# kezakool/flair-for-aigle

Measured on AMD Instinct MI355X. Metric: 512x512x5 tiles/sec (train fwd+bwd+AdamW), U-Net ResNet-34, 19 classes, higher is better.
Workload: dtype bf16; 1 GPU; synthetic 512x512x5 tiles, 19-class U-Net (ResNet-34 encoder), batch 32 per GPU, train step (BASELINE.json configs[1]); global_batch=32, tile=512, parallelism=dp1

## Files before the change

flair-for-aigle_amd/csrc/conv_wgrad.hip:

```cpp
#include "ffa_common.h"
#include <hip/hip_ext.h>

#include <stdlib.h>

#ifndef FFA_WGRAD_TRACE
#define FFA_WGRAD_TRACE 0
#endif
#if FFA_WGRAD_TRACE
__device__ long long ffa_wgrad_trace_buf[64 * 256];
#define FFA_WTRACE(slot_)                                                                   \
  if (trace_on) {                                                                           \
    if (trace_n < 256)                                                                      \
      ffa_wgrad_trace_buf[(blockIdx.y * gridDim.x + blockIdx.x) * 256 + trace_n] =          \
          (long long)(slot_) << 56 | (__builtin_readcyclecounter() & 0xFFFFFFFFFFFFFFLL);    \
    ++trace_n;                                                                              \
  }
#else
#define FFA_WTRACE(slot_)
#endif

struct WgradArgs {
  const void* x;
  const void* dy;
  float* slabs;
  int B, Hi, Wi, Ci;
  int Ho, Wo, Co;
  int pad;
  int tiles_x, tiles_y, npt;
  int ncob, ncib, nsplit;
  const void* x2;
  int C1;
  int CoT, CiT;
  const float* pro_sc;
  const float* pro_sh;
  int ci_real;
};

template <int KH, int KW, int STRIDE, int RG, int WCO, int WCI, int WK, int TH, int TW, int EB>
struct WgradGeom {
  static constexpr int NTHR = 64 * WCO * WCI * WK;
  static constexpr int NPX = TH * TW;
  static constexpr bool ONE = (KH == 1 && KW == 1);
  static constexpr int LS = ONE ? 1 : STRIDE;
  static constexpr int GSTEP = ONE ? STRIDE : 1;
  static constexpr int NRG = KH / RG;
  static constexpr int IH = (TH - 1) * LS + RG;
  static constexpr int IW = (TW - 1) * LS + KW;
  static constexpr int TAPS = RG * KW;
  static constexpr int ROWB = 32 * EB;
  static constexpr int PARTS = ROWB / 16;
  static constexpr int DY_BYTES = WCO * NPX * ROWB;
  static constexpr int IN_BYTES = WCI * IH * IW * ROWB;
  static constexpr int STAGE_BYTES = DY_BYTES + IN_BYTES;
  static constexpr bool MERGE = (WK > 1) && (WCO * WCI == 4 || KH == 7);
  static constexpr int MERGE_BYTES = MERGE ? WCO * WCI * (WK - 1) * TAPS * 16 * 64 * 4 : 0;
  static constexpr int LDS_BYTES = STAGE_BYTES > MERGE_BYTES ? STAGE_BYTES : MERGE_BYTES;
  static constexpr int DY_PIECES = WCO * NPX * PARTS;
  static constexpr int IN_PIECES = WCI * IH * IW * PARTS;
  static constexpr int NDP = (DY_PIECES + NTHR - 1) / NTHR;
  static constexpr int NIP = (IN_PIECES + NTHR - 1) / NTHR;
  static constexpr int KSTEPS = NPX / 16;
  static_assert(TW % 16 == 0, "a 16-pixel k-step must stay inside one tile row");
  static_assert(KSTEPS % WK == 0, "k-steps must divide over the k-split waves");
  static_assert(LDS_BYTES <= 160 * 1024, "LDS budget");
};

__device__ __forceinline__ ffa_s16x4 lds_read_tr16(const unsigned char* p) {
  return __builtin_amdgcn_ds_read_tr16_b64_v4i16(
// ... 1002 lines not shown

  float* slab = a.slabs + (size_t)blockIdx.x * a.CoT * 9 * a.CiT;
#pragma unroll
  for (int mt = 0; mt < MT; ++mt)
#pragma unroll
    for (int nt = 0; nt < NT; ++nt)
#pragma unroll
      for (int tp = 0; tp < 9; ++tp)
#pragma unroll
        for (int i = 0; i < 4; ++i) {
          const int co = mt * 16 + 4 * kg + i, ci = nt * 16 + li;
          slab[((size_t)co * 9 + tp) * a.CiT + ci] = acc[mt][nt][tp][i];
        }
}


template <int TW_>
struct Wg64Geom {
  static constexpr int TW = TW_, TH = 256 / TW_, IH = TH + 2, IW = TW + 2;
  static constexpr int RS = 32 / TW;
  static constexpr int XP = IH * IW * 8, YP = TH * TW * 8;
  static constexpr int PIECES = XP + YP;
  static constexpr int NHW = (PIECES + 511) / 512;
  static constexpr int X_BYTES = XP * 16;
  static constexpr int SLOT = PIECES * 16;
  static constexpr int ACC_BYTES = 144 * 64 * 4;
  static constexpr int LDS_BYTES = (2 * SLOT > 4 * ACC_BYTES) ? 2 * SLOT : 4 * ACC_BYTES;
  static_assert(TW == 32 || TW == 16, "tile width");
  static_assert(LDS_BYTES <= 160 * 1024, "LDS budget");
};

__device__ __forceinline__ int wg64_phi(int px) { return ((px >> 1) & 1) | (((px >> 3) & 1) << 1); }

template <int TW>
__global__ void __launch_bounds__(512) conv3x3_wgrad64_kernel(WgradArgs a) {
  using G = Wg64Geom<TW>;
  __shared__ __align__(16) unsigned char smem[G::LDS_BYTES];
  const int tid = threadIdx.x;
  const int lane = tid & 63;
  const int wave = __builtin_amdgcn_readfirstlane(tid >> 6);
  const int kgp = wave >> 2;
  const int wco = (wave >> 1) & 1, wci = wave & 1;
  const int li = lane & 15, kg = lane >> 4;
  const int cib = blockIdx.x % a.ncib, cob = blockIdx.x / a.ncib;
  const int co0 = cob * 64, ci0 = cib * 64;
  const int split = blockIdx.y;

  const bool two = a.C1 > 0;
  const bool from_lo = two && ci0 < a.C1;
  const size_t xpb = (size_t)(!two ? a.Ci : from_lo ? a.C1 : a.Ci - a.C1) * 2, ypb = (size_t)a.Co * 2;
  const int xW = from_lo ? a.Wi / 2 : a.Wi, xH = from_lo ? a.Hi / 2 : a.Hi;
  int pinfo[G::NHW];
#pragma unroll
  for (int k = 0; k < G::NHW; ++k) {
    const int p = tid + k * 512;
    if (p < G::XP) {
      const int q = p >> 3, yy = q / G::IW, xx = q % G::IW, sl = (p & 7) ^ (2 * wg64_phi(xx));
      const int py = from_lo ? ((yy - 1) >> 1) + 1 : yy, px = from_lo ? ((xx - 1) >> 1) + 1 : xx;
      pinfo[k] = ((((py * xW + px) * (int)xpb) >> 4) + sl) << 13 | (yy << 6) | xx;
    } else if (p < G::PIECES) {
      const int q = (p - G::XP) >> 3, yy = q / G::TW, xx = q % G::TW, sl = (p & 7) ^ (2 * wg64_phi(xx));
      pinfo[k] = ((((yy * a.Wo + xx) * (int)ypb) >> 4) + sl) << 13 | (1 << 12) | (yy << 6) | xx;
    } else {
      pinfo[k] = 1 << 11;
    }
  }
  const unsigned char* x_b = (two && !from_lo) ? static_cast<const unsigned char*>(a.x2) + (ci0 - a.C1) * 2
                                               : static_cast<const unsigned char*>(a.x) + ci0 * 2;
  const unsigned char* dy_b = static_cast<const unsigned char*>(a.dy) + co0 * 2;
  const unsigned char* zero = reinterpret_cast<const unsigned char*>(ffa_wgthin_zero16);
  const bool has_tail = (G::PIECES % 512 == 0) || (wave * 64 + (G::NHW - 1) * 512 < G::PIECES);

  auto tile_origin = [&](int t, int& b, int& oy0, int& ox0) {
    const int tx = t % a.tiles_x;
    const int t2 = t / a.tiles_x;
    oy0 = (t2 % a.tiles_y) * G::TH;
    b = t2 / a.tiles_y;
    ox0 = tx * G::TW;
  };
// ... 98 lines not shown
        __builtin_amdgcn_sched_barrier(0);
      }
      slot ^= 1;
    }
  }
  asm volatile("s_waitcnt vmcnt(0)\n\ts_barrier" ::: "memory");

  float* red = reinterpret_cast<float*>(smem) + (size_t)(wave & 3) * 144 * 64 + lane;
  if (kgp == 1) {
    int o = 0;
#pragma unroll
    for (int mt = 0; mt < 2; ++mt)
#pragma unroll
      for (int nt = 0; nt < 2; ++nt)
#pragma unroll
        for (int tp = 0; tp < 9; ++tp)
#pragma unroll
          for (int i = 0; i < 4; ++i) red[(o++) * 64] = acc[mt][nt][tp][i];
  }
  __syncthreads();
  if (kgp == 1) return;
  {
    int o = 0;
#pragma unroll
    for (int mt = 0; mt < 2; ++mt)
#pragma unroll
      for (int nt = 0; nt < 2; ++nt)
#pragma unroll
        for (int tp = 0; tp < 9; ++tp)
#pragma unroll
          for (int i = 0; i < 4; ++i) acc[mt][nt][tp][i] += red[(o++) * 64];
  }
  float* slab = a.slabs + (size_t)split * a.CoT * 9 * a.CiT;
#pragma unroll
  for (int mt = 0; mt < 2; ++mt)
#pragma unroll
    for (int nt = 0; nt < 2; ++nt)
#pragma unroll
      for (int tp = 0; tp < 9; ++tp)
#pragma unroll
        for (int i = 0; i < 4; ++i) {
          const int co = co0 + wco * 32 + mt * 16 + 4 * kg + i, ci = ci0 + wci * 32 + nt * 16 + li;
          slab[((size_t)co * 9 + tp) * a.CiT + ci] = acc[mt][nt][tp][i];
        }
}


struct WgStem8Geom {
  static constexpr int TH = 8, TW = 32, IH = 2 * TH + 5, IWC = 72;
  static constexpr int XP = IH * IWC, YP = TH * TW * 8;
  static constexpr int PIECES = XP + YP;
  static constexpr int NHW = (PIECES + 511) / 512;
  static constexpr int X_BYTES = XP * 16;
  static constexpr int SLOT = PIECES * 16;
  static constexpr int ACC_BYTES = 112 * 64 * 4;
  static constexpr int LDS_BYTES = (2 * SLOT > 4 * ACC_BYTES) ? 2 * SLOT : 4 * ACC_BYTES;
  static_assert(LDS_BYTES <= 160 * 1024, "LDS budget");
};

__global__ void __launch_bounds__(512) stem_wgrad8_kernel(WgradArgs a) {
  using G = WgStem8Geom;
  __shared__ __align__(16) unsigned char smem[G::LDS_BYTES];
  const int tid = threadIdx.x;
  const int lane = tid & 63;
  const int wave = __builtin_amdgcn_readfirstlane(tid >> 6);
  const int kgp = wave >> 2;
  const int sp = wave & 3;
  const int li = lane & 15, kg = lane >> 4;
  const int split = blockIdx.y;

  int pinfo[G::NHW];
#pragma unroll
  for (int k = 0; k < G::NHW; ++k) {
    const int p = tid + k * 512;
    if (p < G::XP) {
      const int hy = p / G::IWC, hx = p % G::IWC;
      pinfo[k] = (hx < 2 * G::TW + 5) ? (((hy * a.Wi + hx) * 2) << 14 | (hy << 7) | hx) : (1 << 12);
// ... 103 lines not shown
#pragma unroll
      for (int r = 0; r < 7; ++r)
#pragma unroll
        for (int i = 0; i < 4; ++i) red[(o++) * 64] = acc[mt][r][i];
  }
  __syncthreads();
  if (kgp == 1) return;
  {
    int o = 0;
#pragma unroll
    for (int mt = 0; mt < 4; ++mt)
#pragma unroll
      for (int r = 0; r < 7; ++r)
#pragma unroll
        for (int i = 0; i < 4; ++i) acc[mt][r][i] += red[(o++) * 64];
  }
  const int s = 2 * sp + (li >> 3), ch = li & 7;
  if (s < 7) {
#pragma unroll
    for (int mt = 0; mt < 4; ++mt)
#pragma unroll
      for (int r = 0; r < 7; ++r)
#pragma unroll
        for (int i = 0; i < 4; ++i) {
          const int co = mt * 16 + 4 * kg + i;
          a.slabs[(((size_t)split * a.CoT + co) * 49 + r * 7 + s) * 16 + ch] = acc[mt][r][i];
        }
  }
}


struct WgradPlan {
  int wco, wci, wk, th, tw, rg, nsplit, ncob, ncib, CoT, CiT, npt, tiles_x, tiles_y, ring, nslab, stem, thin;
};

static bool wgrad_plan(int dtype, int kh, int kw, int stride, int Co, int Ci, int B, int Ho, int Wo, WgradPlan* p,
                       bool allow_ring = true, bool allow_thin = true) {
  const bool s1 = (kh == 3 && kw == 3 && stride == 1);
  const bool s2 = (kh == 3 && kw == 3 && stride == 2);
  const bool one = (kh == 1 && kw == 1 && (stride == 1 || stride == 2));
  const bool stem = (kh == 7 && kw == 7 && stride == 2);
  if (!(s1 || s2 || one || stem)) return false;
  const bool f32 = (dtype == FFA_F32);
  p->rg = stem ? 1 : kh;
  p->wk = 1;
  p->thin = 0;
  {
    const char* tw_ = getenv("FFA_THIN_WGRAD");
    if (allow_thin && s1 && !f32 && !(tw_ && tw_[0] == '0') && (Co == 16 || Co == 32) && (Ci == 16 || Ci == 32)) {
      p->thin = 1;
      p->th = 8; p->tw = 32;
      p->wco = p->wci = 1;
      p->ncob = p->ncib = 1;
      p->CoT = Co; p->CiT = Ci;
      p->tiles_x = ffa_cdiv(Wo, 32);
      p->tiles_y = ffa_cdiv(Ho, 8);
      p->npt = B * p->tiles_x * p->tiles_y;
      p->ring = 0; p->stem = 0;
      p->nsplit = p->npt < 512 ? p->npt : 512;
      p->nslab = p->nsplit;
      return true;
    }
  }
  if (s1) {
    p->tw = (Wo >= 32) ? 32 : 16;
    p->th = (Wo >= 32) ? 4 : 8;
// ... 46 lines not shown
    p->CoT = Co;
    p->CiT = 16;
    ns = 256 / (Co / 64);
    if (ns > p->npt) ns = p->npt;
    if (ns < 1) ns = 1;
  }
  p->nsplit = ns;
  const bool merge = p->wk > 1 && (p->wco * p->wci == 4 || stem);
  p->nslab = merge ? ns : ns * p->wk;
  return true;
}

extern "C" long long ffa_conv_wgrad_workspace_bytes(int dtype, int kh, int kw, int stride, int Co, int Ci, int B, int Ho,
                                                    int Wo) {
  WgradPlan p, q;
  if (!wgrad_plan(dtype, kh, kw, stride, Co, Ci, B, Ho, Wo, &p)) return FFA_ERR_UNSUPPORTED;
  long long need = (long long)p.nslab * p.CoT * kh * kw * p.CiT * (long long)sizeof(float);
  if (p.thin) {
    wgrad_plan(dtype, kh, kw, stride, Co, Ci, B, Ho, Wo, &q, true, false);
    const long long other = (long long)q.nslab * q.CoT * kh * kw * q.CiT * (long long)sizeof(float);
    if (other > need) need = other;
  }
  return need;
}

template <typename T, int KH, int KW, int STRIDE, int RG, int WCO, int WCI, int WK, int TH, int TW, bool PRO = false>
static void launch_wgrad_cfg(const WgradArgs& a, int nrg, hipStream_t stream) {
  dim3 grid(a.ncob * a.ncib * nrg, a.nsplit);
  hipLaunchKernelGGL((conv_wgrad_kernel<T, KH, KW, STRIDE, RG, WCO, WCI, WK, TH, TW, PRO>), grid,
                     dim3(64 * WCO * WCI * WK), 0, stream, a);
}

template <typename T>
static int launch_wgrad(const WgradArgs& a, const WgradPlan& p, int kh, int kw, int stride, hipStream_t stream) {
  constexpr bool F32 = (sizeof(T) == 4);
  const bool wide = (p.tw == 32);
  if constexpr (!F32) {
    if (p.thin) {
      const bool up = a.C1 > 0, pro = a.pro_sc != nullptr;
#define FFA_WGTHIN(CI_, CO_)                                                                                     \
  if (a.Ci == CI_ && a.Co == CO_) {                                                                              \
    if (up && pro) hipLaunchKernelGGL((conv3x3_thin_wgrad_kernel<CI_, CO_, true, true>), dim3(a.nsplit), dim3(256), 0, stream, a);   \
    else if (up) hipLaunchKernelGGL((conv3x3_thin_wgrad_kernel<CI_, CO_, true, false>), dim3(a.nsplit), dim3(256), 0, stream, a);    \
    else if (pro) hipLaunchKernelGGL((conv3x3_thin_wgrad_kernel<CI_, CO_, false, true>), dim3(a.nsplit), dim3(256), 0, stream, a);   \
    else hipLaunchKernelGGL((conv3x3_thin_wgrad_kernel<CI_, CO_, false, false>), dim3(a.nsplit), dim3(256), 0, stream, a);           \
    return ffa_check_launch("conv3x3_thin_wgrad");                                                               \
  }
      FFA_WGTHIN(16, 16)
      FFA_WGTHIN(16, 32)
      FFA_WGTHIN(32, 16)
      FFA_WGTHIN(32, 32)
#undef FFA_WGTHIN
      ffa_set_error("conv_wgrad: no thin kernel for pitches %d / %d", a.Ci, a.Co);
      return FFA_ERR_UNSUPPORTED;
    }
    if (p.ring) {
      dim3 grid(a.ncob * a.ncib, a.nsplit);
      if (wide) hipLaunchKernelGGL((conv_wgrad_ring_kernel<4, 32>), grid, dim3(256), 0, stream, a);
      else hipLaunchKernelGGL((conv_wgrad_ring_kernel<8, 16>), grid, dim3(256), 0, stream, a);
      return ffa_check_launch("conv_wgrad_ring");
    }
  }
  if (kh == 3 && stride == 1) {
#define FFA_WG_S1(WCO_, WCI_, WK_, THW_, THN_)                                               \
  if (p.wco == WCO_ && p.wci == WCI_ && p.wk == WK_) {                                       \
    if (wide) launch_wgrad_cfg<T, 3, 3, 1, 3, WCO_, WCI_, WK_, THW_, 32>(a, 1, stream);      \
    else launch_wgrad_cfg<T, 3, 3, 1, 3, WCO_, WCI_, WK_, THN_, 16>(a, 1, stream);           \
    return ffa_check_launch("conv_wgrad");                                                   \
  }
    if constexpr (F32) {
      FFA_WG_S1(2, 1, 1, 4, 8)
      FFA_WG_S1(1, 1, 1, 4, 8)
    } else {
      if (a.pro_sc) {
        if (!(p.wco == 2 && p.wci == 2 && p.wk == 2) || a.C1 > 0) {
          ffa_set_error("conv_wgrad: no prologue for this channel configuration");
          return FFA_ERR_UNSUPPORTED;
        }
        if (wide) launch_wgrad_cfg<T, 3, 3, 1, 3, 2, 2, 2, 8, 32, true>(a, 1, stream);
        else launch_wgrad_cfg<T, 3, 3, 1, 3, 2, 2, 2, 16, 16, true>(a, 1, stream);
        return ffa_check_launch("conv_wgrad");
      }
      {
        const char* e64 = getenv("FFA_WGRAD64");
        const int ih = wide ? 10 : 18, iw = wide ? 34 : 18;
        if (!(e64 && e64[0] == '0') && p.wco == 2 && p.wci == 2 && p.wk == 2 && p.th == (wide ? 8 : 16) && a.C1 % 64 == 0 &&
            (a.C1 == 0 || (a.Hi % 2 == 0 && a.Wi % 2 == 0)) && a.pad == 1 && a.Co % 64 == 0 && a.Ci % 64 == 0 &&
            ((long long)ih * a.Wi + iw) * 2 * (a.Ci > a.Co ? a.Ci : a.Co) < (1LL << 23)) {
          hipEvent_t ts, te;
          const dim3 grid(a.ncob * a.ncib, a.nsplit);
          const bool timed = ffa_ktime_next(FFA_KT_WGRAD64, &ts, &te);
          if (wide) {
            if (timed) hipExtLaunchKernelGGL(conv3x3_wgrad64_kernel<32>, grid, dim3(512), 0, stream, ts, te, 0, a);
            else hipLaunchKernelGGL(conv3x3_wgrad64_kernel<32>, grid, dim3(512), 0, stream, a);
          } else {
            if (timed) hipExtLaunchKernelGGL(conv3x3_wgrad64_kernel<16>, grid, dim3(512), 0, stream, ts, te, 0, a);
            else hipLaunchKernelGGL(conv3x3_wgrad64_kernel<16>, grid, dim3(512), 0, stream, a);
          }
          return ffa_check_launch("conv3x3_wgrad64");
        }
      }
      FFA_WG_S1(2, 2, 2, 8, 16)
      FFA_WG_S1(2, 1, 2, 4, 8)
      FFA_WG_S1(1, 2, 2, 4, 8)
      if (p.wco == 1 && p.wci == 1 && p.wk == 4 && (p.th == 8 && wide || p.th == 16 && !wide)) {
        if (wide) launch_wgrad_cfg<T, 3, 3, 1, 3, 1, 1, 4, 8, 32>(a, 1, stream);
        else launch_wgrad_cfg<T, 3, 3, 1, 3, 1, 1, 4, 16, 16>(a, 1, stream);
        return ffa_check_launch("conv_wgrad");
      }
      FFA_WG_S1(1, 1, 4, 4, 8)
    }
#undef FFA_WG_S1
  } else if (kh == 3 && stride == 2) {
    launch_wgrad_cfg<T, 3, 3, 2, 3, 2, F32 ? 1 : 2, 1, 4, 16>(a, 1, stream);
    return ffa_check_launch("conv_wgrad");
  } else if (kh == 1 && stride == 2) {
    launch_wgrad_cfg<T, 1, 1, 2, 1, 2, F32 ? 1 : 2, 1, 4, 16>(a, 1, stream);
    return ffa_check_launch("conv_wgrad");
  } else if (kh == 1 && stride == 1) {
    launch_wgrad_cfg<T, 1, 1, 1, 1, 2, F32 ? 1 : 2, 1, 4, 16>(a, 1, stream);
    return ffa_check_launch("conv_wgrad");
  } else if (kh == 7) {
    if constexpr (!F32) {
// ... 24 lines not shown
              "conv_wgrad: the prologue is for bf16 3x3 stride-1 pad-1 layers");
  FFA_REQUIRE(dtype == FFA_BF16 || dtype == FFA_F32, "conv_wgrad: bad dtype");
  FFA_REQUIRE(x && dy && dw_oihw && workspace, "conv_wgrad: null pointer");
  FFA_REQUIRE(Ci % 8 == 0 && Co % 8 == 0, "conv_wgrad: channel pitch must be a multiple of 8");
  FFA_REQUIRE(Co_real <= Co && Ci_real <= Ci, "conv_wgrad: real channels exceed pitch");
  WgradPlan p;
  const bool thin_ok = pad == 1 && (C1 == 0 || (C1 == Ci && x2 == nullptr));
  if (!wgrad_plan(dtype, kh, kw, stride, Co, Ci, B, Ho, Wo, &p, pad == 1 && C1 == 0, thin_ok)) {
    ffa_set_error("conv_wgrad: unsupported kernel %dx%d stride %d", kh, kw, stride);
    return FFA_ERR_UNSUPPORTED;
  }
  if (C1 > 0 && !p.thin) {
    if (C1 % (32 * p.wci) != 0) {
      ffa_set_error("conv_wgrad_upcat: C1 = %d is not a multiple of the block's %d input channels", C1, 32 * p.wci);
      return FFA_ERR_UNSUPPORTED;
    }
  }
  const long long need = (long long)p.nslab * p.CoT * kh * kw * p.CiT * (long long)sizeof(float);
  if (workspace_bytes < need) {
    ffa_set_error("conv_wgrad: workspace too small (%lld < %lld)", workspace_bytes, need);
    return FFA_ERR_WORKSPACE;
  }
  WgradArgs a;
  a.x = x; a.dy = dy; a.slabs = static_cast<float*>(workspace);
  a.x2 = x2; a.C1 = C1;
  a.pro_sc = pro_scale; a.pro_sh = pro_shift;
  a.ci_real = Ci_real;
  a.B = B; a.Hi = Hi; a.Wi = Wi; a.Ci = Ci;
  a.Ho = Ho; a.Wo = Wo; a.Co = Co;
  a.pad = pad;
  a.tiles_x = p.tiles_x; a.tiles_y = p.tiles_y; a.npt = p.npt;
  a.ncob = p.ncob; a.ncib = p.ncib; a.nsplit = p.nsplit;
  a.CoT = p.CoT; a.CiT = p.CiT;
  int rc = (dtype == FFA_BF16) ? launch_wgrad<ffa_bf16>(a, p, kh, kw, stride, stream)
                               : launch_wgrad<float>(a, p, kh, kw, stride, stream);
  if (rc != FFA_OK) return rc;
  const long long total = (long long)Co_real * kh * kw * ((Ci_real + 3) / 4);
  const char* rv = getenv("FFA_WG_REDUCE_V1");
  const bool reduce_v1 = rv && rv[0] == '1';
  const int cq = (Ci_real + 3) / 4;
  const int v2_blocks = Co_real * ffa_cdiv(cq, p.nslab > 8 ? 8 : 64);
  if (kh == 3 && kw == 3 && !reduce_v1 && v2_blocks >= 512) {
    if (p.nslab > 8) {
      hipLaunchKernelGGL(wgrad_reduce3x3_kernel<32>, dim3(v2_blocks), dim3(256), 0, stream,
                         (const float*)workspace, dw_oihw, p.nslab, p.CoT, p.CiT, Co_real, Ci_real, accumulate);
    } else {
      hipLaunchKernelGGL(wgrad_reduce3x3_kernel<4>, dim3(v2_blocks), dim3(256), 0, stream,
                         (const float*)workspace, dw_oihw, p.nslab, p.CoT, p.CiT, Co_real, Ci_real, accumulate);
    }
    return ffa_check_launch("wgrad_reduce3x3");
  }
  if (p.nslab > 8) {
    long long g = (total + 7) / 8;
    if (g > 4096) g = 4096;
    hipLaunchKernelGGL(wgrad_reduce_kernel<32>, dim3((int)g), dim3(256), 0, stream, (const float*)workspace, dw_oihw,
                       p.nslab, p.CoT, p.CiT, Co_real, Ci_real, kh * kw, accumulate);
  } else {
    long long g = (total + 63) / 64;
    if (g > 4096) g = 4096;
    hipLaunchKernelGGL(wgrad_reduce_kernel<4>, dim3((int)g), dim3(256), 0, stream, (const float*)workspace, dw_oihw,
                       p.nslab, p.CoT, p.CiT, Co_real, Ci_real, kh * kw, accumulate);
  }
  return ffa_check_launch("wgrad_reduce");
}

extern "C" int ffa_conv_wgrad(int dtype, const void* x, const void* dy, float* dw_oihw, int B, int Hi, int Wi, int Ci,
                              int Ho, int Wo, int Co, int Co_real, int Ci_real, int kh, int kw, int stride, int pad,
                              int accumulate, void* workspace, long long workspace_bytes, hipStream_t stream) {
  return wgrad_impl(dtype, x, nullptr, 0, dy, dw_oihw, B, Hi, Wi, Ci, Ho, Wo, Co, Co_real, Ci_real, kh, kw, stride, pad,
// ... 85 lines not shown
```

flair-for-aigle_amd/flairhip/lib.py:

```python
from __future__ import annotations

import ctypes as C
import os

_HERE = os.path.dirname(os.path.abspath(__file__))
LIB_PATH = os.environ.get("FLAIRHIP_LIB") or os.path.join(_HERE, "libflairhip.so")

BF16 = 0
F32 = 1
BCO_RING = 0x1000
BCO_THIN = 0x2000
BCO_STEM = 0x8000
ERR_UNSUPPORTED = -2


class FlairHipError(RuntimeError):
    pass


class Tile(C.Structure):
    _fields_ = [
        ("left", C.c_double), ("bottom", C.c_double), ("right", C.c_double), ("top", C.c_double),
        ("x0", C.c_double), ("y0", C.c_double), ("x1", C.c_double), ("y1", C.c_double),
        ("row", C.c_longlong), ("col", C.c_longlong),
# ... 28 lines not shown
    "ffa_pack_desc_fill_cols": (_i, [_p, _p, _p, _p] + [_i] * 12),
    "ffa_pack_conv_weights_batched": (_i, [_i, _p, _i, _p]),
    "ffa_conv2d": (_i, [_i, _p, _p, _p, _p, _p] + [_i] * 15 + [_p]),
    "ffa_conv_stat_rows": (_ll, [_i, _i, _i, _i, _i]),
    "ffa_conv_plan": (_i, [_i] * 7),
    "ffa_ring_conv3x3": (_i, [_i, _p, _p, _p, _p, _p, _p, _p, _p] + [_i] * 7 + [_p]),
    "ffa_ring_stat_rows": (_ll, [_i, _i, _i, _i]),
    "ffa_ring_pack": (_i, [_i, _p, _p, _p, _i, _i, _i, _i, _i, _p]),
    "ffa_conv2d_pro": (_i, [_i, _p, _p, _p, _p, _p, _p, _p, _p] + [_i] * 9 + [_p]),
    "ffa_conv_wgrad_pro": (_i, [_i, _p, _p, _p, _p, _p] + [_i] * 11 + [_p, _ll, _p]),
    "ffa_thin_eligible": (_i, [_i] * 6),
    "ffa_stem_eligible": (_i, [_i] * 6),
    "ffa_stem_pack_bytes": (_ll, []),
    "ffa_stem_stat_rows": (_ll, [_i, _i, _i]),
    "ffa_stem_pack": (_i, [_p, _p, _p, _i, _i, _p]),
    "ffa_stem_conv7x7": (_i, [_p, _p, _p, _p, _p] + [_i] * 8 + [_p]),
    "ffa_thin_stat_rows": (_ll, [_i, _i, _i, _i]),
    "ffa_thin_conv3x3": (_i, [_p, _p, _p, _p, _p, _p] + [_i] * 9 + [_p]),
    "ffa_thin_conv3x3_pro": (_i, [_p, _p, _p, _p, _p, _p, _p, _p] + [_i] * 9 + [_p]),
    "ffa_thin_pack": (_i, [_p, _p, _p, _i, _i, _i, _i, _i, _p]),
    "ffa_thin_pack_bytes": (_ll, [_i, _i]),
    "ffa_thin_pack_desc_bytes": (_i, []),
    "ffa_thin_pack_desc_fill": (_i, [_p, _p, _p, _p, _i, _i, _i, _i, _i]),
    "ffa_thin_pack_batched": (_i, [_p, _i, _p]),
    "ffa_ring_pack_desc_bytes": (_i, []),
    "ffa_ring_pack_desc_fill": (_i, [_p, _p, _p, _p, _i, _i, _i, _i, _i, _i]),
    "ffa_ring_pack_batched": (_i, [_i, _p, _i, _p]),
    "ffa_conv2d_stats": (_i, [_i, _p, _p, _p, _p, _p, _p] + [_i] * 15 + [_p]),
    "ffa_conv2d_bnbwd": (_i, [_i, _p, _p, _p, _p, _p, _p, _p, _p] + [_i] * 14 + [_p]),
    "ffa_bn_bwd_partials": (_i, [_i, _p, _p, _p, _ll, _p, _p, _p, _p, _p, _p, _p, _ll, _i, _p, _ll, _p]),
    "ffa_conv2d_dgrad_upcat": (_i, [_i, _p, _p, _p, _p] + [_i] * 8 + [_p]),
    "ffa_conv2d_upcat": (_i, [_i, _p, _p, _p, _p, _p, _p] + [_i] * 9 + [_p]),
    "ffa_conv_wgrad_workspace_bytes": (_ll, [_i] * 9),
    "ffa_conv_wgrad": (_i, [_i, _p, _p, _p] + [_i] * 14 + [_p, _ll, _p]),
    "ffa_conv_wgrad_upcat": (_i, [_i, _p, _p, _p, _p] + [_i] * 8 + [_p, _ll, _p]),
    "ffa_conv_is_persistent": (_i, [_i] * 11),
    "ffa_reflect_pad1": (_i, [_i, _p, _p, _i, _i, _i, _i, _p]),
    "ffa_group_norm": (_i, [_i, _p, _p, _p, _p, _p, _ll, _i, _ll, _ll, _i, _ll, _i, _i, _f, _i, _p]),
    "ffa_positional_encoding": (_i, [_p, _p, _i, _i, _i, _f, _p]),
    "ffa_add_rowvec": (_i, [_i, _p, _p, _i, _i, _i, _p]),
    "ffa_ltae_attention": (_i, [_i, _p, _p, _p, _p, _p, _p, _i, _i, _i, _i, _i, _i, _p]),
    "ffa_temporal_aggregate": (_i, [_i, _p, _p, _p, _p, _i, _i, _i, _i, _i, _i, _p]),
    "ffa_detect_pad_images": (_i, [_p, _p, _i, _ll, _f, _p]),
    "ffa_mask_images": (_i, [_i, _p, _p, _i, _ll, _f, _p]),
    "ffa_linear": (_i, [_i, _p, _ll, _p, _p, _p, _ll, _p, _ll, _i, _i, _i, _i, _p]),
    "ffa_space_to_depth": (_i, [_i, _p, _p, _i, _i, _i, _i, _i, _p]),
    "ffa_linear_ex": (_i, [_i, _p, _ll, _p, _p, _p, _ll, _p, _ll, _i, _i, _i, _i, _p, _ll, _p, _i, _p]),
    "ffa_linear_plan": (_i, [_i, _i, _i, _i]),
    "ffa_linear_wgrad_workspace_bytes": (_ll, [_i, _i, _i]),
    "ffa_linear_wgrad": (_i, [_i, _p, _ll, _p, _ll, _p, _p, _i, _i, _i, _i, _p, _ll, _p]),
    "ffa_layer_norm": (_i, [_i, _p, _p, _p, _p, _p, _ll, _i, _f, _p]),
    "ffa_patch_merge_norm": (_i, [_i, _p, _p, _p, _p, _p, _i, _i, _i, _i, _f, _p]),
    "ffa_layer_norm_bwd_workspace_bytes": (_ll, [_ll, _i]),
    "ffa_layer_norm_bwd": (_i, [_i, _p, _p, _p, _p, _p, _p, _p, _p, _ll, _i, _p, _ll, _p]),
    "ffa_scale_rows": (_i, [_i, _p, _p, _p, _ll, _i, _i, _p]),
    "ffa_updown2x_slice": (_i, [_i, _p, _p] + [_i] * 8 + [_p]),
    "ffa_column_sums_workspace_bytes": (_ll, [_ll, _i]),
    "ffa_column_sums": (_i, [_i, _p, _p, _ll, _i, _p, _ll, _p]),
    "ffa_patch_merge_norm_bwd": (_i, [_i, _p, _p, _p, _p, _p, _p, _p, _i, _i, _i, _i, _p, _ll, _p]),
    "ffa_window_attention_bwd_workspace_bytes": (_ll, [_i] * 6),
    "ffa_window_attention_bwd": (_i, [_i, _p, _p, _p, _p, _p, _p, _p, _i, _i, _i, _i, _i, _i, _i, _f, _p, _ll, _p]),
    "ffa_bilinear_slice_bwd": (_i, [_i, _p, _p] + [_i] * 9 + [_p]),
    "ffa_adaptive_avg_pool_bwd": (_i, [_i, _p, _p, _i, _i, _i, _i, _i, _p]),
    "ffa_window_attention": (_i, [_i, _p, _p, _p, _p, _i, _i, _i, _i, _i, _i, _i, _f, _p]),
    "ffa_gelu": (_i, [_i, _p, _p, _ll, _p]),
    "ffa_adaptive_avg_pool": (_i, [_i, _p, _p, _i, _i, _i, _i, _i, _p]),
# ... 93 lines not shown
```

include/flairhip.h:

```cpp
#ifndef FLAIRHIP_H
#define FLAIRHIP_H

#include <stdint.h>

#ifdef __cplusplus
extern "C" {
#endif

typedef struct ihipStream_t* ffa_stream_t;

#define FFA_BF16 0
#define FFA_F32 1

#define FFA_OK 0
#define FFA_ERR_ARG (-1)
#define FFA_ERR_UNSUPPORTED (-2)
#define FFA_ERR_WORKSPACE (-3)

const char* ffa_last_error(void);
int ffa_version(void);
const char* ffa_target_arch(void);


int ffa_conv_block_co(int kh, int kw, int stride, int cout);
// ... 37 lines not shown
int ffa_pack_conv_weight(int dtype, const float* w_oihw, const float* scale, void* dst, int O, int I, int kh, int kw,
                         int transpose, int co_rows, int ci_pitch, int bco, int rg, ffa_stream_t stream);
int ffa_pack_desc_bytes(void);
int ffa_pack_desc_fill(void* host_desc, const float* w_oihw, const float* scale, void* dst, int O, int I, int kh,
                       int kw, int transpose, int co_rows, int ci_pitch, int bco, int rg, int dtype);
int ffa_pack_desc_fill_cols(void* host_desc, const float* w_oihw, const float* scale, void* dst, int O, int I_total,
                            int col0, int ncols, int kh, int kw, int transpose, int co_rows, int ci_pitch, int bco, int rg,
                            int dtype);
int ffa_pack_conv_weights_batched(int dtype, const void* descs_device, int n, ffa_stream_t stream);
int ffa_conv2d(int dtype, const void* in, const void* w_packed, const float* bias, const void* residual, void* out,
               int B, int Hi, int Wi, int Ci, int Ho, int Wo, int Co, int co_rows, int bco, int kh, int kw, int stride,
               int pad, int dil, int relu, ffa_stream_t stream);

long long ffa_conv_stat_rows(int B, int Ho, int Wo, int co_rows, int bco);
int ffa_conv_is_persistent(int dtype, int B, int Ho, int Wo, int Ci, int co_rows, int bco, int kh, int kw, int stride,
                           int dil);
int ffa_conv2d_stats(int dtype, const void* in, const void* w_packed, const float* bias, const void* residual,
                     void* out, float* stat_partials, int B, int Hi, int Wi, int Ci, int Ho, int Wo, int Co,
                     int co_rows, int bco, int kh, int kw, int stride, int pad, int dil, int relu,
                     ffa_stream_t stream);

int ffa_conv2d_bnbwd(int dtype, const void* in, const void* w_packed, const void* residual, void* out,
                     float* stat_partials, const void* bnx, const float* bn_scale, const float* bn_shift, int B, int Hi,
                     int Wi, int Ci, int Ho, int Wo, int Co, int co_rows, int bco, int kh, int kw, int stride, int pad,
                     int dil, ffa_stream_t stream);

int ffa_conv2d_upcat(int dtype, const void* lo, const void* skip, const void* w_packed, const float* bias, void* out,
                     float* stat_partials, int B, int Hl, int Wl, int C1, int C2, int Co, int co_rows, int bco,
                     int relu, ffa_stream_t stream);

int ffa_conv2d_dgrad_upcat(int dtype, const void* dy, const void* w_packed_t, void* dlo, void* dskip, int B, int Ho,
                           int Wo, int Cdy, int C1, int C2, int co_rows, int bco, ffa_stream_t stream);
long long ffa_conv_wgrad_workspace_bytes(int dtype, int kh, int kw, int stride, int Co, int Ci, int B, int Ho, int Wo);
int ffa_conv_wgrad(int dtype, const void* x, const void* dy, float* dw_oihw, int B, int Hi, int Wi, int Ci, int Ho,
                   int Wo, int Co, int Co_real, int Ci_real, int kh, int kw, int stride, int pad, int accumulate,
                   void* workspace, long long workspace_bytes, ffa_stream_t stream);

int ffa_conv_wgrad_upcat(int dtype, const void* lo, const void* skip, const void* dy, float* dw_oihw, int B, int Hl,
                         int Wl, int C1, int C2, int Co, int Co_real, int accumulate, void* workspace,
                         long long workspace_bytes, ffa_stream_t stream);

int ffa_conv2d_pro(int dtype, const void* in, const void* w_packed, const float* bias, const void* residual, void* out,
                   float* stat_partials, const float* pro_scale, const float* pro_shift, int B, int H, int W, int Ci,
                   int Co, int co_rows, int bco, int relu, int up, ffa_stream_t stream);
int ffa_conv_wgrad_pro(int dtype, const void* x, const void* dy, float* dw_oihw, const float* pro_scale,
                       const float* pro_shift, int B, int Hi, int Wi, int Ci, int Ho, int Wo, int Co, int Co_real,
                       int Ci_real, int up, int accumulate, void* workspace, long long workspace_bytes,
                       ffa_stream_t stream);

int ffa_reflect_pad1(int dtype, const void* in, void* out, int N, int H, int W, int C, ffa_stream_t stream);
int ffa_group_norm(int dtype, const void* x, const void* residual, void* y, const float* gamma, const float* beta,
                   long long samples, int Q, long long stride_hi, long long stride_lo, int inner,
                   long long inner_stride, int C, int groups, float eps, int relu, ffa_stream_t stream);
int ffa_positional_encoding(const float* pos, float* out, int n, int d, int repeat, float period, ffa_stream_t stream);
int ffa_add_rowvec(int dtype, void* x, const float* vec, int N, int P, int C, ffa_stream_t stream);
int ffa_ltae_attention(int dtype, const void* k, const void* v, const float* Q, const unsigned char* pad, void* out,
                       float* attn, int B, int T, int P, int n_head, int d_k, int d_v, ffa_stream_t stream);
int ffa_temporal_aggregate(int dtype, const void* x, const float* attn, const unsigned char* pad, void* out, int B,
                           int T, int P, int C, int n_head, int use_pad, ffa_stream_t stream);
int ffa_detect_pad_images(const float* x, unsigned char* pad, int N, long long per_image, float value,
                          ffa_stream_t stream);
int ffa_mask_images(int dtype, void* x, const unsigned char* pad, int N, long long per_image, float value,
                    ffa_stream_t stream);
int ffa_reflect_pad1_bwd(int dtype, const void* dpad, void* dx, int N, int H, int W, int C, ffa_stream_t stream);
int ffa_group_norm_bwd(int dtype, const void* x, const void* dy, void* dx, const float* gamma, const float* beta,
                       float* partial, long long samples, int Q, long long stride_hi, long long stride_lo, int inner,
// ... 219 lines not shown
```

Baseline: 2400 tiles/s.

## Write wgrad64 partials as per-wave tiles and reduce with dedicated tile kernels

The 3x3 wgrad64 kernel now stores each wave's accumulator fragment as contiguous float4 vectors in a tiled slab layout instead of scattered OIHW-order scalar stores. It uses a 1-D grid with a block remap that interleaves splits across channel blocks. New row and tile reduction kernels sum the splits and scatter into dw, chosen by split count. The goal is coalesced partial-sum writes and reads and better block spreading across the device. The old path stays behind FFA_WGRAD64_V1.

```diff
diff --git a/flair-for-aigle_amd/csrc/conv_wgrad.hip b/flair-for-aigle_amd/csrc/conv_wgrad.hip
--- a/flair-for-aigle_amd/csrc/conv_wgrad.hip
+++ b/flair-for-aigle_amd/csrc/conv_wgrad.hip
@@ -34,6 +34,7 @@
   const float* pro_sc;
   const float* pro_sh;
   int ci_real;
+  int w64_v1;
 };
 
 template <int KH, int KW, int STRIDE, int RG, int WCO, int WCI, int WK, int TH, int TW, int EB>
@@ -1102,6 +1103,20 @@
 
 __device__ __forceinline__ int wg64_phi(int px) { return ((px >> 1) & 1) | (((px >> 3) & 1) << 1); }
 
+__host__ __device__ inline int wg64_block_map(int L, int nb) {
+  const int full = (nb / 8) * 8;
+  return L < full ? (L % 8) * (full / 8) + L / 8 : L;
+}
+
+extern "C" void ffa_wgrad64_block_map(int nb, int* out) {
+  for (int L = 0; L < nb; ++L) out[L] = wg64_block_map(L, nb);
+}
+
+struct Wg64Slab {
+  static constexpr int ROW = 64 * 4;
+  static constexpr int TILE = 36 * 64;
+};
+
 template <int TW>
 __global__ void __launch_bounds__(512) conv3x3_wgrad64_kernel(WgradArgs a) {
   using G = Wg64Geom<TW>;
@@ -1112,9 +1127,11 @@
   const int kgp = wave >> 2;
   const int wco = (wave >> 1) & 1, wci = wave & 1;
   const int li = lane & 15, kg = lane >> 4;
-  const int cib = blockIdx.x % a.ncib, cob = blockIdx.x / a.ncib;
+  const int ncb = a.ncob * a.ncib;
+  const int item = a.w64_v1 ? (int)(blockIdx.y * ncb + blockIdx.x) : wg64_block_map(blockIdx.x, gridDim.x);
+  const int cb = item % ncb, split = item / ncb;
+  const int cib = cb % a.ncib, cob = cb / a.ncib;
   const int co0 = cob * 64, ci0 = cib * 64;
-  const int split = blockIdx.y;
 
   const bool two = a.C1 > 0;
   const bool from_lo = two && ci0 < a.C1;
@@ -1279,17 +1296,131 @@
           for (int i = 0; i < 4; ++i) acc[mt][nt][tp][i] += red[(o++) * 64];
   }
   float* slab = a.slabs + (size_t)split * a.CoT * 9 * a.CiT;
+  if (a.w64_v1) {
+#pragma unroll
+    for (int mt = 0; mt < 2; ++mt)
+#pragma unroll
+      for (int nt = 0; nt < 2; ++nt)
+#pragma unroll
+        for (int tp = 0; tp < 9; ++tp)
+#pragma unroll
+          for (int i = 0; i < 4; ++i) {
+            const int co = co0 + wco * 32 + mt * 16 + 4 * kg + i, ci = ci0 + wci * 32 + nt * 16 + li;
+            slab[((size_t)co * 9 + tp) * a.CiT + ci] = acc[mt][nt][tp][i];
+          }
+    return;
+  }
+  float* mine = slab + ((size_t)cb * 4 + (wave & 3)) * (Wg64Slab::TILE * 4) + lane * 4;
 #pragma unroll
   for (int mt = 0; mt < 2; ++mt)
 #pragma unroll
     for (int nt = 0; nt < 2; ++nt)
 #pragma unroll
       for (int tp = 0; tp < 9; ++tp)
-#pragma unroll
-        for (int i = 0; i < 4; ++i) {
-          const int co = co0 + wco * 32 + mt * 16 + 4 * kg + i, ci = ci0 + wci * 32 + nt * 16 + li;
-          slab[((size_t)co * 9 + tp) * a.CiT + ci] = acc[mt][nt][tp][i];
-        }
+        *reinterpret_cast<ffa_f32x4*>(mine + ((mt * 2 + nt) * 9 + tp) * Wg64Slab::ROW) = acc[mt][nt][tp];
+}
+
+template <int SL, int LT>
+__global__ void __launch_bounds__(576)
+wgrad64_reduce_tile_kernel(const float* __restrict__ slabs, float* __restrict__ dw, int nsplit, int CoT, int CiT, int ncib,
+                           int Co, int Ci, int accumulate) {
+  constexpr int NH = SL / LT, PP = 64 / NH, NCO = 16 / NH;
+  static_assert(LT % 8 == 0 || LT == 4, "batches of eight");
+  __shared__ __align__(16) float out[9 * PP * 4];
+  const int tile = blockIdx.x / NH, ph = blockIdx.x % NH, cb = tile >> 4, T = tile & 15;
+  const int co_base = (cb / ncib) * 64 + (T >> 3) * 32 + ((T >> 1) & 1) * 16 + ph * NCO;
+  const int ci_base = (cb % ncib) * 64 + ((T >> 2) & 1) * 32 + (T & 1) * 16;
+  if (co_base >= Co || ci_base >= Ci) return;
+  const int tap = threadIdx.x >> 6, pl = threadIdx.x & (PP - 1), h = (threadIdx.x & 63) / PP;
+  const size_t slab = (size_t)CoT * 9 * CiT;
+  const float* src = slabs + ((size_t)tile * 9 + tap) * Wg64Slab::ROW + (ph * PP + pl) * 4;
+  ffa_f32x4 s[LT];
+#pragma unroll
+  for (int l = 0; l < LT; ++l) s[l] = ffa_f32x4{0.f, 0.f, 0.f, 0.f};
+  for (int k0 = h * LT; k0 < nsplit; k0 += (LT == 4 ? 8 : SL)) {
+#pragma unroll
+    for (int b = 0; b < (LT == 4 ? 8 : LT); b += 8) {
+      ffa_f32x4 v[8];
+#pragma unroll
+      for (int u = 0; u < 8; ++u) {
+        const int k = k0 + b + u;
+        const ffa_f32x4 t = *reinterpret_cast<const ffa_f32x4*>(src + (size_t)(k < nsplit ? k : k0) * slab);
+        v[u] = k < nsplit ? t : ffa_f32x4{0.f, 0.f, 0.f, 0.f};
+      }
+#pragma unroll
+      for (int u = 0; u < 8; ++u)
+#pragma unroll
+        for (int e = 0; e < 4; ++e) s[(b + u) % LT][e] += v[u][e];
+    }
+  }
+  ffa_f32x4 t = ffa_f32x4{0.f, 0.f, 0.f, 0.f};
+  ffa_f32x4* mine = reinterpret_cast<ffa_f32x4*>(out) + tap * PP + pl;
+#pragma unroll
+  for (int hh = 0; hh < NH; ++hh) {
+    if (hh > 0) {
+      __syncthreads();
+      if (h == hh) t = *mine;
+    }
+    if (h == hh) {
+#pragma unroll
+      for (int l = 0; l < LT; ++l)
+#pragma unroll
+        for (int e = 0; e < 4; ++e) t[e] += s[l][e];
+      *mine = t;
+    }
+  }
+  __syncthreads();
+  const int nci = min(16, Ci - ci_base), nco = min(NCO, Co - co_base);
+  for (int o = threadIdx.x; o < NCO * 144; o += 576) {
+    const int c = o / 144, rem = o % 144, li = rem / 9, tp = rem % 9;
+    if (c < nco && li < nci) {
+      float* dst = dw + ((size_t)(co_base + c) * Ci + ci_base) * 9 + rem;
+      const float r = out[(tp * PP + (c >> 2) * 16 + li) * 4 + (c & 3)];
+      *dst = accumulate ? (*dst + r) : r;
+    }
+  }
+}
+
+__global__ void __launch_bounds__(1024)
+wgrad64_reduce_row_kernel(const float* __restrict__ slabs, float* __restrict__ dw, int nsplit, int CoT, int CiT, int ncib,
+                          int Co, int Ci, int accumulate) {
+  constexpr int SL = 32;
+  __shared__ __align__(16) float sh[SL * Wg64Slab::ROW];
+  const int row = blockIdx.x, tile = row / 9, tap = row % 9, cb = tile >> 4, T = tile & 15;
+  const int co_base = (cb / ncib) * 64 + (T >> 3) * 32 + ((T >> 1) & 1) * 16;
+  const int ci_base = (cb % ncib) * 64 + ((T >> 2) & 1) * 32 + (T & 1) * 16;
+  if (co_base >= Co || ci_base >= Ci) return;
+  const int g = threadIdx.x >> 6, pos = threadIdx.x & 63;
+  const size_t slab = (size_t)CoT * 9 * CiT;
+  const float* src = slabs + (size_t)row * Wg64Slab::ROW + pos * 4;
+  ffa_f32x4 s[2] = {ffa_f32x4{0.f, 0.f, 0.f, 0.f}, ffa_f32x4{0.f, 0.f, 0.f, 0.f}};
+  for (int k0 = g; k0 < nsplit; k0 += 8 * 16) {
+    ffa_f32x4 v[8];
+#pragma unroll
+    for (int u = 0; u < 8; ++u) {
+      const int k = k0 + u * 16;
+      const ffa_f32x4 t = *reinterpret_cast<const ffa_f32x4*>(src + (size_t)(k < nsplit ? k : k0) * slab);
+      v[u] = k < nsplit ? t : ffa_f32x4{0.f, 0.f, 0.f, 0.f};
+    }
+#pragma unroll
+    for (int u = 0; u < 8; ++u)
+#pragma unroll
+      for (int e = 0; e < 4; ++e) s[u & 1][e] += v[u][e];
+  }
+  *reinterpret_cast<ffa_f32x4*>(sh + g * Wg64Slab::ROW + pos * 4) = s[0];
+  *reinterpret_cast<ffa_f32x4*>(sh + (g + 16) * Wg64Slab::ROW + pos * 4) = s[1];
+  __syncthreads();
+  if (threadIdx.x < 256) {
+    const int c = threadIdx.x >> 4, li = threadIdx.x & 15;
+    const float* col = sh + ((c >> 2) * 16 + li) * 4 + (c & 3);
+    float t = 0.f;
+#pragma unroll 8
+    for (int l = 0; l < SL; ++l) t += col[l * Wg64Slab::ROW];
+    if (co_base + c < Co && ci_base + li < Ci) {
+      float* dst = dw + ((size_t)(co_base + c) * Ci + ci_base + li) * 9 + tap;
+      *dst = accumulate ? (*dst + t) : t;
+    }
+  }
 }
 
 
@@ -1459,6 +1590,7 @@
 
 struct WgradPlan {
   int wco, wci, wk, th, tw, rg, nsplit, ncob, ncib, CoT, CiT, npt, tiles_x, tiles_y, ring, nslab, stem, thin;
+  int slab64;
 };
 
 static bool wgrad_plan(int dtype, int kh, int kw, int stride, int Co, int Ci, int B, int Ho, int Wo, WgradPlan* p,
@@ -1571,7 +1703,8 @@
 }
 
 template <typename T>
-static int launch_wgrad(const WgradArgs& a, const WgradPlan& p, int kh, int kw, int stride, hipStream_t stream) {
+static int launch_wgrad(const WgradArgs& a, WgradPlan& p, int kh, int kw, int stride, hipStream_t stream) {
+  p.slab64 = 0;
   constexpr bool F32 = (sizeof(T) == 4);
   const bool wide = (p.tw == 32);
   if constexpr (!F32) {
@@ -1627,7 +1760,8 @@
             (a.C1 == 0 || (a.Hi % 2 == 0 && a.Wi % 2 == 0)) && a.pad == 1 && a.Co % 64 == 0 && a.Ci % 64 == 0 &&
             ((long long)ih * a.Wi + iw) * 2 * (a.Ci > a.Co ? a.Ci : a.Co) < (1LL << 23)) {
           hipEvent_t ts, te;
-          const dim3 grid(a.ncob * a.ncib, a.nsplit);
+          const dim3 grid = a.w64_v1 ? dim3(a.ncob * a.ncib, a.nsplit) : dim3(a.ncob * a.ncib * a.nsplit);
+          p.slab64 = a.w64_v1 ? 0 : 1;
           const bool timed = ffa_ktime_next(FFA_KT_WGRAD64, &ts, &te);
           if (wide) {
             if (timed) hipExtLaunchKernelGGL(conv3x3_wgrad64_kernel<32>, grid, dim3(512), 0, stream, ts, te, 0, a);
@@ -1718,9 +1852,26 @@
   a.tiles_x = p.tiles_x; a.tiles_y = p.tiles_y; a.npt = p.npt;
   a.ncob = p.ncob; a.ncib = p.ncib; a.nsplit = p.nsplit;
   a.CoT = p.CoT; a.CiT = p.CiT;
+  const char* w1 = getenv("FFA_WGRAD64_V1");
+  a.w64_v1 = (w1 && w1[0] == '1') ? 1 : 0;
   int rc = (dtype == FFA_BF16) ? launch_wgrad<ffa_bf16>(a, p, kh, kw, stride, stream)
                                : launch_wgrad<float>(a, p, kh, kw, stride, stream);
   if (rc != FFA_OK) return rc;
+  if (p.slab64) {
+    const int tiles = p.ncob * p.ncib * 16;
+    const float* ws = (const float*)workspace;
+    if (p.nslab >= 64) {
+      hipLaunchKernelGGL(wgrad64_reduce_row_kernel, dim3(tiles * 9), dim3(1024), 0, stream, ws, dw_oihw, p.nslab, p.CoT,
+                         p.CiT, p.ncib, Co_real, Ci_real, accumulate);
+    } else if (p.nslab > 8) {
+      hipLaunchKernelGGL((wgrad64_reduce_tile_kernel<32, 16>), dim3(tiles * 2), dim3(576), 0, stream, ws, dw_oihw, p.nslab, p.CoT,
+                         p.CiT, p.ncib, Co_real, Ci_real, accumulate);
+    } else {
+      hipLaunchKernelGGL((wgrad64_reduce_tile_kernel<4, 4>), dim3(tiles), dim3(576), 0, stream, ws, dw_oihw, p.nslab, p.CoT,
+                         p.CiT, p.ncib, Co_real, Ci_real, accumulate);
+    }
+    return ffa_check_launch("wgrad64_reduce");
+  }
   const long long total = (long long)Co_real * kh * kw * ((Ci_real + 3) / 4);
   const char* rv = getenv("FFA_WG_REDUCE_V1");
   const bool reduce_v1 = rv && rv[0] == '1';
diff --git a/flair-for-aigle_amd/flairhip/lib.py b/flair-for-aigle_amd/flairhip/lib.py
--- a/flair-for-aigle_amd/flairhip/lib.py
+++ b/flair-for-aigle_amd/flairhip/lib.py
@@ -84,6 +84,7 @@
     "ffa_conv2d_dgrad_upcat": (_i, [_i, _p, _p, _p, _p] + [_i] * 8 + [_p]),
     "ffa_conv2d_upcat": (_i, [_i, _p, _p, _p, _p, _p, _p] + [_i] * 9 + [_p]),
     "ffa_conv_wgrad_workspace_bytes": (_ll, [_i] * 9),
+    "ffa_wgrad64_block_map": (None, [_i, _p]),
     "ffa_conv_wgrad": (_i, [_i, _p, _p, _p] + [_i] * 14 + [_p, _ll, _p]),
     "ffa_conv_wgrad_upcat": (_i, [_i, _p, _p, _p, _p] + [_i] * 8 + [_p, _ll, _p]),
     "ffa_conv_is_persistent": (_i, [_i] * 11),
diff --git a/include/flairhip.h b/include/flairhip.h
--- a/include/flairhip.h
+++ b/include/flairhip.h
@@ -93,6 +93,7 @@
 int ffa_conv2d_dgrad_upcat(int dtype, const void* dy, const void* w_packed_t, void* dlo, void* dskip, int B, int Ho,
                            int Wo, int Cdy, int C1, int C2, int co_rows, int bco, ffa_stream_t stream);
 long long ffa_conv_wgrad_workspace_bytes(int dtype, int kh, int kw, int stride, int Co, int Ci, int B, int Ho, int Wo);
+void ffa_wgrad64_block_map(int nb, int* out);
 int ffa_conv_wgrad(int dtype, const void* x, const void* dy, float* dw_oihw, int B, int Hi, int Wi, int Ci, int Ho,
                    int Wo, int Co, int Co_real, int Ci_real, int kh, int kw, int stride, int pad, int accumulate,
                    void* workspace, long long workspace_bytes, ffa_stream_t stream);
```

Result: no change. 2388 tiles/s (-0.5%).
